# 1005088h/3d_object_detection

Hardware: AMD Instinct MI355X
Metric: point-cloud frames/sec end-to-end (voxelise→NMS), eight_20cm, 1x MI355X (higher is better)
Workload: dtype f32; 1 GPU; configs/eight_20cm.json, synthetic KITTI-shape 64-beam 20k-point clouds (mean 20000 points, one distinct cloud per frame of a step), independent frames (batch=1 semantics), random-init weights (InstanceNorm backbone), AABB NMS; `value`: clouds resident in HBM; frames_per_pass_per_gpu=32, engine_max_batch=32, parallelism=frame-sharded x1

## Files before the change

3d_object_detection_amd/_lib.py:

```python
import ctypes
import os

_HERE = os.path.dirname(os.path.abspath(__file__))
LIB_PATH = os.path.join(_HERE, "csrc", "libpp_hip.so")
PP_MAX_CLASSES = 12
PP_LOSS_TERMS = 21
PP_ASSIGN_MAX_GT = 4096
PP_AUG_MAX_BOXES = 256
PP_AUG_MAX_TRIES = 128
PP_AUG_PARAMS = 16

c_f = ctypes.c_float
c_i32 = ctypes.c_int32
c_i64 = ctypes.c_int64
c_p = ctypes.c_void_p


class PPConfig(ctypes.Structure):
    _fields_ = [
        ("voxel_size", c_f * 3),
        ("offset", c_f * 3),
        ("grid_size", c_i32 * 3),
        ("max_voxels", c_i32),
        ("max_num_points", c_i32),
# ... 23 lines not shown
    "pp_effective_precision": (ctypes.c_int, [c_p]),
    "pp_set_anchors": (ctypes.c_int, [c_p, c_p, c_p, c_i64]),
    "pp_voxelize": (ctypes.c_int, [c_p, c_p, ctypes.c_int, ctypes.c_int, c_p, c_p, c_p, c_p, c_p]),
    "pp_anchor_mask": (ctypes.c_int, [c_p, c_p, c_p, c_p, c_p]),
    "pp_pfn": (ctypes.c_int, [c_p, c_p, c_p, c_p, c_p, c_p, c_p]),
    "pp_scatter": (ctypes.c_int, [c_p, c_p, c_p, c_p, c_p, c_p]),
    "pp_backbone": (ctypes.c_int, [c_p, c_p, c_p, c_p]),
    "pp_head": (ctypes.c_int, [c_p, c_p, c_p, c_p, c_p, c_p]),
    "pp_postprocess": (ctypes.c_int, [c_p, c_p, c_p, c_p, c_p, c_p, c_p, ctypes.c_int, c_p]),
    "pp_select_candidates": (ctypes.c_int, [c_p, c_p, c_p, c_p, c_p, c_p, c_p, c_p, c_p]),
    "pp_infer_frame": (ctypes.c_int, [c_p, c_p, ctypes.c_int, c_p, c_p, ctypes.c_int, c_p]),
    "pp_infer_batch": (ctypes.c_int, [c_p, ctypes.POINTER(c_p), ctypes.POINTER(c_i32), ctypes.c_int, c_p, c_p, ctypes.c_int, c_p]),
    "pp_fetch_frame_tensor": (ctypes.c_int, [c_p, ctypes.c_int, ctypes.c_int, c_p, c_p]),
    "pp_set_head_defer": (ctypes.c_int, [c_p, ctypes.c_int]),
    "pp_head_defer_active": (ctypes.c_int, [c_p]),
    "pp_set_assign_thresholds": (ctypes.c_int, [c_p, c_p, c_p]),
    "pp_assign_targets": (ctypes.c_int, [c_p, c_p, c_p, c_p, ctypes.POINTER(c_i32), ctypes.c_int, c_p, c_p, c_p, c_p, c_p]),
    "pp_target_loss": (ctypes.c_int, [c_p, c_p, c_p, c_p, c_p, c_p, c_p, ctypes.c_int, c_p, c_p]),
    "pp_batch_loss": (ctypes.c_int, [c_p, c_p, c_p, ctypes.POINTER(c_i32), ctypes.c_int, c_p, c_p]),
    "pp_target_loss_grad": (ctypes.c_int, [c_p, c_p, c_p, c_p, c_p, c_p, c_p, ctypes.c_int, ctypes.c_int, c_f, c_p, c_p, c_p, c_p]),
    "pp_head_backward": (ctypes.c_int, [c_p, c_p, c_p, c_p, c_p, ctypes.c_int, c_p, c_p, c_p, c_p, c_p, c_p, c_p, c_p]),
    "pp_update_head_weights": (ctypes.c_int, [c_p, c_p, c_p, c_p, c_p, c_p, c_p, c_p]),
    "pp_augment_draw": (ctypes.c_int, [c_p, ctypes.c_uint64, ctypes.c_uint32, ctypes.POINTER(c_i64), ctypes.c_int, ctypes.c_int,
                                       ctypes.POINTER(c_i32), ctypes.c_int, c_p, c_p, c_p, c_p, c_p]),
    "pp_augment_noise": (ctypes.c_int, [c_p, c_p, c_p, c_p, c_p, c_p, ctypes.c_int, ctypes.POINTER(c_i32), ctypes.c_int, c_p, c_p, c_p, c_p]),
    "pp_augment_boxes": (ctypes.c_int, [c_p, c_p, c_p, c_p, c_p, c_p, c_p, c_p, ctypes.POINTER(c_i32), ctypes.c_int, c_p, c_p, c_p, c_p, c_p]),
    "pp_augment_points": (ctypes.c_int, [c_p, c_p, c_p, ctypes.POINTER(c_i32), c_p, c_p, c_p, c_p, c_p, ctypes.POINTER(c_i32), ctypes.c_int,
                                         c_p, c_p]),
    "pp_box_decode": (ctypes.c_int, [c_p, c_p, c_p, c_i64, c_p]),
    "pp_corners2d": (ctypes.c_int, [c_p, c_p, c_p, c_p, c_i64, c_p]),
# ... 48 lines not shown
```

3d_object_detection_amd/csrc/conv.hip:

```cpp
#include <algorithm>
#include <type_traits>
#include <cmath>
#include <cstdio>
#include <cstdlib>
#include <cstring>
#include <unistd.h>
#include "pp_common.h"
#include "conv_common.h"

namespace {

using namespace ppc;

template <int KS, int STRIDE, int TW, int WM, int WN, int MT, int NT, int BTX, int KC, int EPI>
struct ConvCfg {
    static constexpr int TH = 16 / TW;
    static constexpr int TILES = WN * NT;
    static constexpr int BTY = TILES / BTX;
    static constexpr int PW = BTX * TW, PH = BTY * TH;
    static constexpr int IW = (PW - 1) * STRIDE + KS, IH = (PH - 1) * STRIDE + KS;
    static constexpr int HALF = (IW + 1) / 2;
    static constexpr int iwp()
    {
        int v = IW;
// ... 2796 lines not shown
        for (Layer& L : net->layers) {
            int rc = 0;
            {
                const int h = H >> L.level, w = W >> L.level;
                const int hin = (L.kind == 0 && L.stride == 2) ? h * 2 : h, win = (L.kind == 0 && L.stride == 2) ? w * 2 : w;
                if (!can_tune && net->eff_prec == 0) L.var = pick_variant(L.kind, L.stride, L.up, (L.kind == 2) ? head_rows(ctx->cfg.num_anchor_per_loc) : (L.kind == 1 ? L.cout * L.up * L.up : L.cout), h, w, ctx->cfg.num_anchor_per_loc == 9);
                rc = autotune_layer(ctx, L, hin, win, h, w, tin, tout, verbose, can_tune);
                if (rc) { if (tin) { (void)hipFree(tin - W6_FRONT_PAD); (void)hipFree(tout); } return rc; }
            }
            PP_HIP(hipFuncSetAttribute((const void*)L.var.kern, hipFuncAttributeMaxDynamicSharedMemorySize,
                                       (int)layer_lds(L.var, L.cin)));
            if (L.var.kern2) PP_HIP(hipFuncSetAttribute((const void*)L.var.kern2, hipFuncAttributeMaxDynamicSharedMemorySize, (int)L.var.lds));
            rc = pack_layer(ctx, L);
            if (rc) { if (tin) { (void)hipFree(tin - W6_FRONT_PAD); (void)hipFree(tout); } return rc; }
        }
        {
            const Layer& head = net->layers.back();
            net->defer_ok = net->eff_prec == 0 && na == 9 && head.var.family == Family::Gemm1x1 && head.var.prec == 0 && head.var.io16 == 0;
            if (net->defer_ok) {
                const int rc = autotune_head_cls(ctx, tin, verbose, can_tune);
                if (rc) { if (tin) { (void)hipFree(tin - W6_FRONT_PAD); (void)hipFree(tout); } return rc; }
            }
        }
        if (tin) { PP_HIP(hipDeviceSynchronize()); (void)hipFree(tin - W6_FRONT_PAD); (void)hipFree(tout); tune_cache_save(); }
        if (net->up16)
            for (const Layer& L : net->layers)
                if ((L.kind == 1 && L.var.io16 != 3) || (L.kind == 2 && L.var.io16 != 1) ||
                    (L.kind == 0 && L.var.io16 != ((L.stride == 2 && L.level == 0) ? 2 : 3)))
                    return pp_fail(ctx, PP_E_STATE, "fp16s: a layer did not get a 16-bit-tensor tiling (PP_FORCE_VARIANT?)");
    }
// ... 73 lines not shown
    if (bx > 64) bx = 64;
    hipLaunchKernelGGL(norm_relu_stats, dim3(bx, C, B), dim3(256), 0, stream, x, y, C, HW, pre.mode, pre.acc, pre.scale,
                       pre.shift, pre.inv_n, 1e-3f, stat, (size_t)C * HW, STAT_FS, x16, y16);
    PP_HIP(hipGetLastError());
    return 0;
}

}

int pp_run_backbone(pp_ctx* ctx, const float* canvas, int nb, hipStream_t stream, const int32_t* pmap, const float* feat)
{
    pp_net* net = (pp_net*)ctx->net;
    const int H = ctx->H, W = ctx->W;
    if ((H % 4) || (W % 4)) return pp_fail(ctx, PP_E_ARG, "backbone: BEV grid must be a multiple of 8 in x and y");
    if (nb < 1 || nb > ctx->max_batch) return pp_fail(ctx, PP_E_ARG, "backbone: batch exceeds cfg.max_batch");
    if (ctx->cfg.norm_kind == 0) PP_HIP(hipMemsetAsync(net->stats, 0, STAT_FS * sizeof(double) * nb, stream));
    NormRef raw;
    const float* x = canvas;
    int Hin = ctx->gx, Win = ctx->gy;
    size_t li = 0;
    const int up_coff[3] = {0, 64, 192};
    const size_t up_fs = (size_t)320 * H * W;
    for (int b = 0; b < 3; ++b) {
        const int c = kC[b];
        const int h = H >> b, w = W >> b;
        const size_t cnt = (size_t)h * w;
        float** Bf = net->buf[b];
        int rc;
        if ((rc = launch_conv(ctx, net->layers[li++], x, Hin, Win, Bf[0], nullptr, raw, stat_slot(ctx, site_block(b, 0)), c, h, w, stream,
                              nullptr, nullptr, nb, 0, 0, b == 0 ? pmap : nullptr, b == 0 ? feat : nullptr))) return rc;
        if ((rc = pp_stage_mark(ctx, stream, PP_ST_NORM))) return rc;
        if ((rc = launch_norm_relu(ctx, Bf[0], Bf[1], c, (int)cnt, norm_ref(ctx, site_block(b, 0), c, 0, cnt),
                                   stat_slot(ctx, site_block(b, 1)), stream, nb, net->up16 ? 1 : 0, net->up16 ? 1 : 0))) return rc;
        if ((rc = pp_stage_mark(ctx, stream, PP_ST_CONV))) return rc;
        float* cur = Bf[1];
        float* spare[3] = {Bf[0], Bf[2], Bf[3]};
        const int nunits = (b == 0) ? 2 : 3;
        for (int u = 0; u < nunits; ++u) {
            const int nl = (u == nunits - 1) ? 0 : 1;
            const bool last = (u == nunits - 1);
            float* t1 = spare[0];
            float* t2 = spare[1];
            double* out_stat = last ? nullptr : stat_slot(ctx, site_block(b, 1 + 2 * (u + 1)));
            if (nl == 1) {
// ... 180 lines not shown
    switch (kind) {
    case 0: src = ctx->f_cls + frame * A; bytes = A * 4; break;
    case 1: src = ctx->f_box + frame * A * 7; bytes = A * 28; break;
    case 2: src = ctx->f_dir + frame * A * 2; bytes = A * 8; break;
    case 3: src = ctx->f_mask + frame * A; bytes = A; break;
    case 4: {
        NormRef pre = norm_ref(ctx, 7, 320, 0, HW);
        if (pre.mode == PRE_STATS) pre.acc += (size_t)frame * STAT_FS;
        const float* src_ = net->up16 ? reinterpret_cast<const float*>(reinterpret_cast<const _Float16*>(net->up) + (size_t)frame * 320 * HW)
                                      : net->up + (size_t)frame * 320 * HW;
        return launch_norm_relu(ctx, src_, (float*)dst, 320, (int)HW, pre, nullptr, stream, 1, net->up16 ? 1 : 0);
    }
    case 5: src = ctx->f_feat + frame * mv * 64; bytes = mv * 64 * 4; break;
    case 6: src = ctx->f_coors + frame * mv * 3; bytes = mv * 12; break;
    case 7: src = ctx->f_num + frame * 4; bytes = 4; break;
    default: return pp_fail(ctx, PP_E_ARG, "pp_fetch_frame_tensor: unknown kind");
    }
    PP_HIP(hipMemcpyAsync(dst, src, bytes, hipMemcpyDeviceToDevice, stream));
    return 0;
}

extern "C" int pp_profile_begin(pp_ctx* ctx)
{
    if (!ctx) return PP_E_ARG;
    ctx->prof_on = true;
    ctx->prof_used = 0;
    return 0;
}

extern "C" int pp_profile_end(pp_ctx* ctx, double* avg_ms, int32_t* launches, double* flops)
// ... 92 lines not shown
```

3d_object_detection_amd/csrc/pp_api.hip:

```cpp
#include <cmath>
#include <cstdio>
#include <cstdlib>
#include <cstring>
#include "pp_common.h"

static std::string g_create_err;

int pp_fail_hip(pp_ctx* ctx, hipError_t e, const char* what, const char* file, int line)
{
    char buf[512];
    snprintf(buf, sizeof(buf), "%s failed: %s (%s:%d)", what, hipGetErrorString(e), file, line);
    if (ctx) ctx->err = buf; else g_create_err = buf;
    (void)hipGetLastError();
    return -(int)e;
}

int pp_fail(pp_ctx* ctx, int code, const char* msg)
{
    if (ctx) ctx->err = msg; else g_create_err = msg;
    return code;
}

extern "C" const char* pp_last_error(pp_ctx* ctx) { return ctx ? ctx->err.c_str() : g_create_err.c_str(); }
extern "C" int pp_version(void) { return 4; }
// ... 77 lines not shown
    PP_HIP(dalloc(&ctx->f_voxels, mv * c.max_num_points * c.num_point_features));
    PP_HIP(dalloc(&ctx->f_coors, mv * 3));
    PP_HIP(dalloc(&ctx->f_npts, mv));
    PP_HIP(dalloc(&ctx->f_num, 4 * (size_t)ctx->max_batch));
    PP_HIP(dalloc(&ctx->f_feat, mv * 64));
    PP_HIP(dalloc(&ctx->f_canvas, (size_t)64 * ctx->gx * ctx->gy));
    PP_HIP(dalloc(&ctx->f_pmap, (size_t)ctx->max_batch * ctx->gx * ctx->gy));
    size_t HW = (size_t)ctx->H * ctx->W;
    size_t Amax = HW * c.num_anchor_per_loc * ctx->max_batch;
    PP_HIP(dalloc(&ctx->f_mask, Amax));
    PP_HIP(dalloc(&ctx->f_cls, Amax));
    PP_HIP(dalloc(&ctx->f_box, Amax * 7));
    PP_HIP(dalloc(&ctx->f_dir, Amax * 2));
    int rc = pp_net_create(ctx);
    if (rc) return rc;
    rc = pp_post_create(ctx);
    return rc;
}

extern "C" pp_ctx* pp_create(int device, const pp_config* cfg)
{
    if (!cfg) { pp_fail(nullptr, PP_E_ARG, "pp_create: null config"); return nullptr; }
    if (cfg->grid_size[2] != 1 || cfg->grid_size[0] < 2 || cfg->grid_size[1] < 2 || (cfg->grid_size[0] & 1) ||
        (cfg->grid_size[1] & 1)) {
        pp_fail(nullptr, PP_E_ARG, "pp_create: grid must be [gx,gy,1] with even gx,gy (multiples of 8 for the backbone)");
        return nullptr;
    }
    if (cfg->max_voxels <= 0 || cfg->max_num_points <= 0 || cfg->max_points <= 0 || cfg->num_classes <= 0 ||
        cfg->num_classes > PP_MAX_CLASSES || cfg->nms_pre_max <= 0 || cfg->nms_pre_max > 4096 ||
        cfg->nms_post_max <= 0 || cfg->nms_post_max > cfg->nms_pre_max || cfg->nms_post_max > 1024 || cfg->max_batch < 0 ||
        cfg->max_batch > 64) {
        pp_fail(nullptr, PP_E_ARG, "pp_create: size out of range");
        return nullptr;
    }
    pp_ctx* ctx = new pp_ctx();
    ctx->cfg = *cfg;
    ctx->max_batch = cfg->max_batch > 0 ? cfg->max_batch : 1;
    ctx->cfg.max_batch = ctx->max_batch;
    ctx->device = device;
    ctx->gx = cfg->grid_size[0];
    ctx->gy = cfg->grid_size[1];
    ctx->H = ctx->gx / 2;
    ctx->W = ctx->gy / 2;
    if (const char* e = getenv("PP_HEAD_DEFER")) ctx->head_defer_env_off = e[0] == '0';
    ctx->head_defer = !ctx->head_defer_env_off;
    int rc = create_impl(ctx);
    if (rc) {
        g_create_err = ctx->err;
        pp_destroy(ctx);
        return nullptr;
    }
    return ctx;
}

int pp_build_tables(pp_ctx* ctx)
{
    if (ctx->tab_A == ctx->A) return 0;
    const pp_config& c = ctx->cfg;
    const size_t mv = (size_t)c.max_voxels;
    const size_t vs = mv * c.max_num_points * c.num_point_features;
// ... 16 lines not shown
        pp_post_frame& q = post[b];
        PP_SET(q.cls, ctx->f_cls + b * A); PP_SET(q.box, ctx->f_box + b * A * 7); PP_SET(q.dir, ctx->f_dir + b * A * 2); PP_SET(q.mask, ctx->f_mask + b * A);
        pp_post_fill_table(ctx, b, &q);
    }
    PP_HIP(hipMemcpy(ctx->d_pre, pre.data(), sizeof(pp_pre_frame) * pre.size(), hipMemcpyHostToDevice));
    PP_HIP(hipMemcpy(ctx->d_post, post.data(), sizeof(pp_post_frame) * post.size(), hipMemcpyHostToDevice));
    ctx->tab_A = ctx->A;
    return 0;
}

extern "C" void pp_destroy(pp_ctx* ctx)
{
    if (!ctx) return;
    (void)hipSetDevice(ctx->device);
    pp_net_destroy(ctx);
    pp_post_destroy(ctx);
    pp_assign_destroy(ctx);
    pp_train_destroy(ctx);
    for (pp_slot& S : ctx->slot) {
        void* sp[] = {S.cell_first, S.pt_cell, S.pt_rank, S.wave_cnt, S.occ};
        for (void* q : sp)
            if (q) (void)hipFree(q);
    }
    if (ctx->d_pre) (void)hipFree(ctx->d_pre);
    if (ctx->d_post) (void)hipFree(ctx->d_post);
    void* ptrs[] = {ctx->anchors, ctx->rect_x, ctx->rect_y, ctx->rects, ctx->pfn_w, ctx->pfn_scale, ctx->pfn_shift,
                    ctx->f_voxels, ctx->f_coors, ctx->f_npts, ctx->f_num, ctx->f_feat, ctx->f_canvas, ctx->f_mask, ctx->f_pmap,
                    ctx->f_cls, ctx->f_box, ctx->f_dir};
    for (void* p : ptrs)
        if (p) (void)hipFree(p);
// ... 43 lines not shown
                      *b = find_w(ctx, p + "1.bias", 64), *rm = find_w(ctx, p + "1.running_mean", 64),
                      *rv = find_w(ctx, p + "1.running_var", 64);
    if (!w || !g || !b || !rm || !rv) return pp_fail(ctx, PP_E_NAME, "pp_commit_weights: PFN tensors missing or mis-shaped");
    float wT[9 * 64], sc[64], sh[64];
    for (int c = 0; c < 64; ++c) {
        for (int k = 0; k < 9; ++k) wT[k * 64 + c] = w->data[c * 9 + k];
        double s = (double)g->data[c] / std::sqrt((double)rv->data[c] + 1e-5);
        sc[c] = (float)s;
        sh[c] = (float)((double)b->data[c] - (double)rm->data[c] * s);
    }
    PP_HIP(hipMemcpy(ctx->pfn_w, wT, sizeof(wT), hipMemcpyHostToDevice));
    PP_HIP(hipMemcpy(ctx->pfn_scale, sc, sizeof(sc), hipMemcpyHostToDevice));
    PP_HIP(hipMemcpy(ctx->pfn_shift, sh, sizeof(sh), hipMemcpyHostToDevice));
    int rc = pp_net_commit(ctx);
    if (rc) return rc;
    ctx->weights_ready = true;
    ++ctx->commit_gen;
    return 0;
}

extern "C" int pp_set_anchors(pp_ctx* ctx, const float* anchors_h, const int32_t* rects_h, int64_t A)
{
    if (!ctx || !anchors_h || !rects_h || A <= 0) return pp_fail(ctx, PP_E_ARG, "pp_set_anchors: bad argument");
    PP_HIP(hipSetDevice(ctx->device));
    const int H = ctx->H, W = ctx->W;
    const int64_t HW = (int64_t)H * W;
    if (A % HW != 0 || A / HW != ctx->cfg.num_anchor_per_loc)
        return pp_fail(ctx, PP_E_ARG, "pp_set_anchors: A must be num_anchor_per_loc * (gx/2) * (gy/2)");
    for (int i = 0; i < 4 * A; ++i) {
        int lim = (i & 1) ? ctx->gy : ctx->gx;
// ... 31 lines not shown
```

3d_object_detection_amd/csrc/pp_common.h:

```cpp
#pragma once
#include <hip/hip_runtime.h>
#include <stdint.h>
#include <map>
#include <string>
#include <vector>
#include "../../include/pp_hip.h"

#define PP_EMPTY 0x7F7F7F7F

#define PP_HIP(call)                                                         \
    do {                                                                     \
        hipError_t e_ = (call);                                              \
        if (e_ != hipSuccess) return pp_fail_hip(ctx, e_, #call, __FILE__, __LINE__); \
    } while (0)

#if defined(__HIP_DEVICE_COMPILE__)
#define PP_GP __attribute__((address_space(1)))
#else
#define PP_GP
#endif
#define PP_SET(dst, src) dst = (decltype(dst))(src)
struct pp_pre_frame {
    int32_t PP_GP *pt_cell, *cell_first, *wave_cnt, *pt_rank, *slots, *scalars, *occ;
    float PP_GP* voxels;
// ... 74 lines not shown
    std::vector<hipEvent_t> stage_ev;
    std::vector<int> stage_id;
    std::vector<hipStream_t> stage_stream;
    size_t stage_used = 0;
    int last_nb = 0;
    bool asg_thr_set = false;
    float asg_thr_m[PP_MAX_CLASSES] = {}, asg_thr_u[PP_MAX_CLASSES] = {};
    void* asg = nullptr;
    uint64_t commit_gen = 0;
    void* trn = nullptr;
    bool head_defer = true;
    bool head_defer_env_off = false;
    bool head_stale = false;
    int stale_nb = 0;
    hipStream_t stale_stream = nullptr;
};
enum { PP_ST_VOXELIZE = 0, PP_ST_MASK = 1, PP_ST_PFN = 2, PP_ST_CONV = 3, PP_ST_NORM = 4, PP_ST_HEAD = 5, PP_ST_POST = 6 ,
       PP_ST_POST_TOPK = 7 , PP_ST_POST_NMS = 8 , PP_ST_COUNT = 12 };
int pp_stage_mark(pp_ctx* ctx, hipStream_t stream, int id);

int pp_fail_hip(pp_ctx* ctx, hipError_t e, const char* what, const char* file, int line);
int pp_fail(pp_ctx* ctx, int code, const char* msg);

int pp_net_create(pp_ctx* ctx);
void pp_net_destroy(pp_ctx* ctx);
int pp_net_commit(pp_ctx* ctx);
int pp_post_create(pp_ctx* ctx);
int pp_voxelize_slot(pp_ctx* ctx, int s, const float* pts, int n, int nfeat, float* voxels, int32_t* coors, int32_t* npts,
                     int32_t* num_pillars, hipStream_t stream);
int pp_anchor_mask_slot(pp_ctx* ctx, int s, const int32_t* coors, const int32_t* num_pillars, uint8_t* mask, hipStream_t stream);
// ... 7 lines not shown
int pp_anchor_mask_group(pp_ctx* ctx, int b0, int g, hipStream_t stream);
int pp_pfn_pmap_group(pp_ctx* ctx, int b0, int g, hipStream_t stream);
int pp_postprocess_group(pp_ctx* ctx, int b0, int g, float* det, int32_t* det_count, int nms_mode, hipStream_t stream,
                         int defer_nb = 0);
int pp_run_head_fused(pp_ctx* ctx, float* cls, float* box, float* dir, int nb, hipStream_t stream);
bool pp_head_defer_on(pp_ctx* ctx);
int pp_run_head_cls(pp_ctx* ctx, float* cls, int nb, hipStream_t stream);
int pp_head_materialise(pp_ctx* ctx, hipStream_t stream);
struct pp_head_gather {
    const float* w; int bm, bmp, K;
    const float* bias_perm;
    const float* in; size_t in_fs; int HW;
    int pre; const double* pre_acc; size_t pre_fs; double pre_inv_n; const float *pre_scale, *pre_shift; size_t aff_fs; float eps;
};
int pp_net_head_gather(pp_ctx* ctx, int nb, pp_head_gather* g);
void pp_post_destroy(pp_ctx* ctx);
void pp_assign_destroy(pp_ctx* ctx);
void pp_train_destroy(pp_ctx* ctx);
struct pp_head_image {
    float *w = nullptr, *bias = nullptr, *bias_perm = nullptr;
    std::vector<int32_t> wmap, bmap, bpmap;
};
int pp_net_head_image(pp_ctx* ctx, pp_head_image* img);

static inline int pp_div_up(int64_t a, int64_t b) { return (int)((a + b - 1) / b); }
```

3d_object_detection_amd/engine.py:

```python
import ctypes
import os
import weakref

import numpy as np
import torch

from . import _lib

F32 = np.float32

DETECT_CLASSES = ["vehicle", "pedestrian", "cyclist"]
CLASS_TABLE = {
    "vehicle": dict(sizes=[[4.6, 2.10, 1.8], [7.5, 2.6, 2.9], [12.6, 2.9, 3.8]], rotations=[0, 1.5707963267948966],
                    matched_threshold=0.6, unmatched_threshold=0.45),
    "pedestrian": dict(sizes=[[0.96874749, 0.9645992, 1.81212425]], rotations=[0],
                       matched_threshold=0.45, unmatched_threshold=0.25),
    "cyclist": dict(sizes=[[2.02032733, 0.98075615, 1.72027404]], rotations=[0, 1.5707963267948966],
                    matched_threshold=0.5, unmatched_threshold=0.25),
}
NUM_ANCHOR_PER_LOC = 9


def class_table_of(config):
    tab = config.get("class_table")
# ... 178 lines not shown
        if changed and self.weights_loaded:
            with torch.cuda.device(self.device):
                _lib.check(self.lib.pp_commit_weights(self.ctx), self.ctx, "pp_commit_weights")

    def effective_precision(self):
        v = self.lib.pp_effective_precision(self.ctx)
        return None if v < 0 else {n: k for k, n in self.PRECISIONS.items()}[v]

    def set_head_defer(self, on):
        _lib.check(self.lib.pp_set_head_defer(self.ctx, 1 if on else 0), self.ctx, "pp_set_head_defer")
        self.head_defer = bool(on) and not self._defer_env_off

    def head_defer_active(self):
        return bool(self.lib.pp_head_defer_active(self.ctx))

    def load_state_dict(self, sd):
        for k, v in sd.items():
            if k.endswith("num_batches_tracked"):
                continue
            a = v.detach().cpu().numpy() if isinstance(v, torch.Tensor) else np.asarray(v)
            a = np.ascontiguousarray(a, dtype=F32)
            shape = (ctypes.c_int64 * max(a.ndim, 1))(*a.shape)
            _lib.check(self.lib.pp_load_weights(self.ctx, k.encode(), a.ctypes.data_as(ctypes.c_void_p), shape, a.ndim),
                       self.ctx, "pp_load_weights(" + k + ")")
        with torch.cuda.device(self.device):
            _lib.check(self.lib.pp_commit_weights(self.ctx), self.ctx, "pp_commit_weights")
        self.weights_loaded = True

    def _t(self, shape, dtype):
        return torch.empty(shape, dtype=dtype, device=self.device)
# ... 157 lines not shown
        rows = self.cfg.num_classes * self.cfg.nms_post_max
        if det is None:
            det = torch.zeros((nb, rows, 9), dtype=torch.float32, device=self.device)
            cnt = torch.zeros((nb, 1 + _lib.PP_MAX_CLASSES), dtype=torch.int32, device=self.device)
        ptrs = (ctypes.c_void_p * nb)(*[p.data_ptr() if p.numel() else _ptr(p).value for p in points_list])
        ns = (ctypes.c_int32 * nb)(*[int(p.shape[0]) for p in points_list])
        with torch.cuda.device(self.device):
            _lib.check(self.lib.pp_infer_batch(self.ctx, ptrs, ns, nb, _ptr(det), _ptr(cnt), int(nms_mode), _stream()),
                       self.ctx, "pp_infer_batch")
        return det, cnt

    def fetch(self, frame, what):
        kinds = {"cls": (0, (self.A,), torch.float32), "box": (1, (self.A, 7), torch.float32), "dir": (2, (self.A, 2), torch.float32),
                 "mask": (3, (self.A,), torch.uint8), "rpn": (4, (320, self.H, self.W), torch.float32),
                 "feat": (5, (self.max_voxels, 64), torch.float32), "coors": (6, (self.max_voxels, 3), torch.int32),
                 "num": (7, (1,), torch.int32)}
        kind, shape, dtype = kinds[what]
        out = torch.empty(shape, dtype=dtype, device=self.device)
        with torch.cuda.device(self.device):
            _lib.check(self.lib.pp_fetch_frame_tensor(self.ctx, int(frame), kind, _ptr(out), _stream()), self.ctx, "pp_fetch_frame_tensor")
        return out

    def _gt_args(self, gt_boxes, gt_classes, gt_offsets, nb, what):
        G = int(gt_boxes.shape[0]) if gt_boxes.dim() == 2 else -1
        gt_boxes = _chk(gt_boxes, torch.float32, (G, 7), what + ": gt_boxes")
        gt_classes = _chk(gt_classes, torch.int32, (G,), what + ": gt_classes")
        off = [int(v) for v in gt_offsets]
        if not 1 <= nb <= self.max_batch:
            raise ValueError(f"{what}: {nb} frames, max_batch is {self.max_batch}")
        if len(off) != nb + 1 or off[0] != 0 or off[-1] != G or any(b < a for a, b in zip(off, off[1:])):
            raise ValueError(f"{what}: gt offsets must be {nb + 1} non-decreasing values from 0 to {G}")
# ... 248 lines not shown
```

include/pp_hip.h:

```cpp
#ifndef PP_HIP_H
#define PP_HIP_H
#include <stdint.h>

#ifdef __cplusplus
extern "C" {
#endif

#define PP_MAX_CLASSES 12
#define PP_E_ARG 1
#define PP_E_STATE 2
#define PP_E_NAME 3

typedef struct pp_ctx pp_ctx;

typedef struct pp_config {
    float voxel_size[3];
    float offset[3];
    int32_t grid_size[3];
    int32_t max_voxels;
    int32_t max_num_points;
    int32_t num_point_features;
    int32_t max_points;
    int32_t num_anchor_per_loc;
    int32_t num_classes;
// ... 40 lines not shown

int pp_select_candidates(pp_ctx* ctx, const float* cls, const float* box, const float* dir, const uint8_t* mask,
                         int32_t* idx, float* score, int32_t* count, void* stream);

int pp_infer_frame(pp_ctx* ctx, const float* pts, int n, float* det, int32_t* det_count, int nms_mode, void* stream);

#define PP_DET_COUNT_STRIDE (1 + PP_MAX_CLASSES)
int pp_infer_batch(pp_ctx* ctx, const float* const* pts_h, const int32_t* n_h, int nb, float* det, int32_t* det_count,
                   int nms_mode, void* stream);

int pp_fetch_frame_tensor(pp_ctx* ctx, int frame, int kind, void* dst, void* stream);

int pp_set_head_defer(pp_ctx* ctx, int on);
int pp_head_defer_active(pp_ctx* ctx);

#define PP_ASSIGN_MAX_GT 4096
#define PP_LOSS_TERMS 21
int pp_set_assign_thresholds(pp_ctx* ctx, const float* matched_h, const float* unmatched_h);
int pp_assign_targets(pp_ctx* ctx, const uint8_t* mask, const float* gt, const int32_t* gt_cls, const int32_t* gt_off_h, int nb,
                      int32_t* labels, float* bbox_targets, float* outside_w, int32_t* dir_targets, void* stream);
int pp_target_loss(pp_ctx* ctx, const float* cls, const float* box, const float* dir, const int32_t* labels,
                   const float* bbox_targets, const int32_t* dir_targets, int nb, double* terms, void* stream);
int pp_batch_loss(pp_ctx* ctx, const float* gt, const int32_t* gt_cls, const int32_t* gt_off_h, int nb, double* terms, void* stream);

int pp_target_loss_grad(pp_ctx* ctx, const float* cls, const float* box, const float* dir, const int32_t* labels,
                        const float* bbox_targets, const int32_t* dir_targets, int nb, int batch_div, float grad_scale, float* dcls,
                        float* dbox, float* ddir, void* stream);
int pp_head_backward(pp_ctx* ctx, const float* rpn_out, const float* dcls, const float* dbox, const float* ddir, int nb, float* dw_cls,
                     float* dw_box, float* dw_dir, float* db_cls, float* db_box, float* db_dir, float* dx, void* stream);
int pp_update_head_weights(pp_ctx* ctx, const float* w_cls, const float* b_cls, const float* w_box, const float* b_box, const float* w_dir,
// ... 58 lines not shown
```

Measured before the change: 1012 frames/s.

## Add sparse gather-based first backbone conv over active output pixels

Replaces the dense stride-2 3x3 first backbone convolution with a sparse path. It ballots the output pixels whose receptive field contains an occupied pillar, compacts them into a per-frame list with gather tables, and runs an MFMA kernel that reads pillar features straight from the voxel feature buffer. It writes only the active outputs after zeroing the output plane, and accumulates the norm statistics inside the same kernel. The path is on by default for fp32 and adds three launches plus a memset, with results capped at a fixed active-pixel capacity.

```diff
diff --git a/3d_object_detection_amd/_lib.py b/3d_object_detection_amd/_lib.py
--- a/3d_object_detection_amd/_lib.py
+++ b/3d_object_detection_amd/_lib.py
@@ -61,6 +61,7 @@
     "pp_fetch_frame_tensor": (ctypes.c_int, [c_p, ctypes.c_int, ctypes.c_int, c_p, c_p]),
     "pp_set_head_defer": (ctypes.c_int, [c_p, ctypes.c_int]),
     "pp_head_defer_active": (ctypes.c_int, [c_p]),
+    "pp_set_sparse_conv1": (ctypes.c_int, [c_p, ctypes.c_int]),
     "pp_set_assign_thresholds": (ctypes.c_int, [c_p, c_p, c_p]),
     "pp_assign_targets": (ctypes.c_int, [c_p, c_p, c_p, c_p, ctypes.POINTER(c_i32), ctypes.c_int, c_p, c_p, c_p, c_p, c_p]),
     "pp_target_loss": (ctypes.c_int, [c_p, c_p, c_p, c_p, c_p, c_p, c_p, ctypes.c_int, c_p, c_p]),
diff --git a/3d_object_detection_amd/csrc/conv.hip b/3d_object_detection_amd/csrc/conv.hip
--- a/3d_object_detection_amd/csrc/conv.hip
+++ b/3d_object_detection_amd/csrc/conv.hip
@@ -2834,6 +2834,7 @@
             rc = pack_layer(ctx, L);
             if (rc) { if (tin) { (void)hipFree(tin - W6_FRONT_PAD); (void)hipFree(tout); } return rc; }
         }
+        ctx->sc1_kc = (net->layers[0].var.family == Family::Direct && net->layers[0].var.kc == 8) ? 8 : 4;
         {
             const Layer& head = net->layers.back();
             net->defer_ok = net->eff_prec == 0 && na == 9 && head.var.family == Family::Gemm1x1 && head.var.prec == 0 && head.var.io16 == 0;
@@ -2937,6 +2938,7 @@
     const int H = ctx->H, W = ctx->W;
     if ((H % 4) || (W % 4)) return pp_fail(ctx, PP_E_ARG, "backbone: BEV grid must be a multiple of 8 in x and y");
     if (nb < 1 || nb > ctx->max_batch) return pp_fail(ctx, PP_E_ARG, "backbone: batch exceeds cfg.max_batch");
+    ctx->sc1_last_nb = 0;
     if (ctx->cfg.norm_kind == 0) PP_HIP(hipMemsetAsync(net->stats, 0, STAT_FS * sizeof(double) * nb, stream));
     NormRef raw;
     const float* x = canvas;
@@ -2950,7 +2952,10 @@
         const size_t cnt = (size_t)h * w;
         float** Bf = net->buf[b];
         int rc;
-        if ((rc = launch_conv(ctx, net->layers[li++], x, Hin, Win, Bf[0], nullptr, raw, stat_slot(ctx, site_block(b, 0)), c, h, w, stream,
+        if (b == 0 && pmap && net->eff_prec == 0 && pp_sc1_usable(ctx)) {
+            ++li;
+            if ((rc = pp_sc1_run(ctx, pmap, feat, Bf[0], stat_slot(ctx, site_block(0, 0)), STAT_FS, nb, stream))) return rc;
+        } else if ((rc = launch_conv(ctx, net->layers[li++], x, Hin, Win, Bf[0], nullptr, raw, stat_slot(ctx, site_block(b, 0)), c, h, w, stream,
                               nullptr, nullptr, nb, 0, 0, b == 0 ? pmap : nullptr, b == 0 ? feat : nullptr))) return rc;
         if ((rc = pp_stage_mark(ctx, stream, PP_ST_NORM))) return rc;
         if ((rc = launch_norm_relu(ctx, Bf[0], Bf[1], c, (int)cnt, norm_ref(ctx, site_block(b, 0), c, 0, cnt),
@@ -3161,6 +3166,7 @@
     case 5: src = ctx->f_feat + frame * mv * 64; bytes = mv * 64 * 4; break;
     case 6: src = ctx->f_coors + frame * mv * 3; bytes = mv * 12; break;
     case 7: src = ctx->f_num + frame * 4; bytes = 4; break;
+    case 8: return pp_sc1_fetch_list(ctx, frame, dst, stream);
     default: return pp_fail(ctx, PP_E_ARG, "pp_fetch_frame_tensor: unknown kind");
     }
     PP_HIP(hipMemcpyAsync(dst, src, bytes, hipMemcpyDeviceToDevice, stream));
diff --git a/3d_object_detection_amd/csrc/pp_api.hip b/3d_object_detection_amd/csrc/pp_api.hip
--- a/3d_object_detection_amd/csrc/pp_api.hip
+++ b/3d_object_detection_amd/csrc/pp_api.hip
@@ -115,6 +115,8 @@
     PP_HIP(dalloc(&ctx->f_dir, Amax * 2));
     int rc = pp_net_create(ctx);
     if (rc) return rc;
+    rc = pp_sc1_create(ctx);
+    if (rc) return rc;
     rc = pp_post_create(ctx);
     return rc;
 }
@@ -145,6 +147,8 @@
     ctx->W = ctx->gy / 2;
     if (const char* e = getenv("PP_HEAD_DEFER")) ctx->head_defer_env_off = e[0] == '0';
     ctx->head_defer = !ctx->head_defer_env_off;
+    if (const char* e = getenv("PP_SPARSE_CONV1")) ctx->sparse_conv1_env_off = e[0] == '0';
+    ctx->sparse_conv1 = !ctx->sparse_conv1_env_off;
     int rc = create_impl(ctx);
     if (rc) {
         g_create_err = ctx->err;
@@ -191,6 +195,7 @@
     if (!ctx) return;
     (void)hipSetDevice(ctx->device);
     pp_net_destroy(ctx);
+    pp_sc1_destroy(ctx);
     pp_post_destroy(ctx);
     pp_assign_destroy(ctx);
     pp_train_destroy(ctx);
@@ -264,6 +269,7 @@
     PP_HIP(hipMemcpy(ctx->pfn_shift, sh, sizeof(sh), hipMemcpyHostToDevice));
     int rc = pp_net_commit(ctx);
     if (rc) return rc;
+    if ((rc = pp_sc1_commit(ctx))) return rc;
     ctx->weights_ready = true;
     ++ctx->commit_gen;
     return 0;
diff --git a/3d_object_detection_amd/csrc/pp_common.h b/3d_object_detection_amd/csrc/pp_common.h
--- a/3d_object_detection_amd/csrc/pp_common.h
+++ b/3d_object_detection_amd/csrc/pp_common.h
@@ -112,6 +112,11 @@
     bool head_stale = false;
     int stale_nb = 0;
     hipStream_t stale_stream = nullptr;
+    bool sparse_conv1 = true;
+    bool sparse_conv1_env_off = false;
+    void* sc1 = nullptr;
+    int sc1_kc = 4;
+    int sc1_last_nb = 0;
 };
 enum { PP_ST_VOXELIZE = 0, PP_ST_MASK = 1, PP_ST_PFN = 2, PP_ST_CONV = 3, PP_ST_NORM = 4, PP_ST_HEAD = 5, PP_ST_POST = 6 ,
        PP_ST_POST_TOPK = 7 , PP_ST_POST_NMS = 8 , PP_ST_COUNT = 12 };
@@ -149,6 +154,12 @@
     int pre; const double* pre_acc; size_t pre_fs; double pre_inv_n; const float *pre_scale, *pre_shift; size_t aff_fs; float eps;
 };
 int pp_net_head_gather(pp_ctx* ctx, int nb, pp_head_gather* g);
+int pp_sc1_create(pp_ctx* ctx);
+void pp_sc1_destroy(pp_ctx* ctx);
+int pp_sc1_commit(pp_ctx* ctx);
+bool pp_sc1_usable(pp_ctx* ctx);
+int pp_sc1_run(pp_ctx* ctx, const int32_t* pmap, const float* feat, float* out, double* stat, size_t stat_fs, int nb, hipStream_t stream);
+int pp_sc1_fetch_list(pp_ctx* ctx, int frame, void* dst, hipStream_t stream);
 void pp_post_destroy(pp_ctx* ctx);
 void pp_assign_destroy(pp_ctx* ctx);
 void pp_train_destroy(pp_ctx* ctx);
diff --git a/3d_object_detection_amd/csrc/sparse_conv1.hip b/3d_object_detection_amd/csrc/sparse_conv1.hip
--- /dev/null
+++ b/3d_object_detection_amd/csrc/sparse_conv1.hip
@@ -0,0 +1,317 @@
+#include <algorithm>
+#include <cstring>
+#include "pp_common.h"
+#include "conv_common.h"
+
+namespace {
+
+using namespace ppc;
+
+constexpr unsigned SC1_PARK = 0x80000000u;
+constexpr int SC1_NT = 4;
+constexpr int SC1_WAVE_PX = 16 * SC1_NT;
+constexpr int SC1_W_FLOATS = 9 * 64 * 64;
+
+struct Sc1 {
+    float* w = nullptr;
+    int kc = 4;
+    uint64_t* words = nullptr;
+    int32_t* bcnt = nullptr;
+    int32_t* list = nullptr;
+    uint32_t* tab = nullptr;
+    int32_t* count = nullptr;
+    int cap = 0, cap_pad = 0, nblk = 0;
+    bool weights = false;
+};
+
+struct Sc1P {
+    const int32_t* pmap; size_t pmap_fs;
+    const float* feat; size_t feat_fs; unsigned feat_bytes;
+    const float* w;
+    float* out; size_t out_fs;
+    double* stat; size_t stat_fs;
+    uint64_t* words; int32_t* bcnt; int32_t* list; uint32_t* tab; int32_t* count;
+    int Hin, Win, Hout, Wout, cap, cap_pad, nblk, max_voxels;
+};
+
+__global__ void __launch_bounds__(256) sc1_ballot_b(const Sc1P p)
+{
+    __shared__ int wc[4];
+    const int f = blockIdx.z;
+    const int32_t* __restrict__ gmap = p.pmap + (size_t)f * p.pmap_fs;
+    const int pix = blockIdx.x * 256 + threadIdx.x;
+    bool act = false;
+    if (pix < p.Hout * p.Wout) {
+        const int oy = pix / p.Wout, ox = pix - oy * p.Wout;
+#pragma unroll
+        for (int ky = 0; ky < 3; ++ky) {
+            const int iy = 2 * oy - 1 + ky;
+#pragma unroll
+            for (int kx = 0; kx < 3; ++kx) {
+                const int ix = 2 * ox - 1 + kx;
+                if (iy >= 0 && iy < p.Hin && ix >= 0 && ix < p.Win) act |= gmap[(size_t)iy * p.Win + ix] >= 0;
+            }
+        }
+    }
+    const uint64_t b = __ballot(act);
+    const int wave = threadIdx.x >> 6;
+    if ((threadIdx.x & 63) == 0) {
+        p.words[((size_t)f * p.nblk + blockIdx.x) * 4 + wave] = b;
+        wc[wave] = __popcll(b);
+    }
+    __syncthreads();
+    if (threadIdx.x == 0) p.bcnt[(size_t)f * p.nblk + blockIdx.x] = wc[0] + wc[1] + wc[2] + wc[3];
+}
+
+__global__ void __launch_bounds__(256) sc1_write_b(const Sc1P p)
+{
+    __shared__ int red[4];
+    const int f = blockIdx.z, blk = blockIdx.x, tid = threadIdx.x, lane = tid & 63, wave = tid >> 6;
+    const uint64_t* __restrict__ wd = p.words + ((size_t)f * p.nblk + blk) * 4;
+    const int32_t* __restrict__ bc = p.bcnt + (size_t)f * p.nblk;
+    const uint64_t w0 = wd[0], w1 = wd[1], w2 = wd[2], w3 = wd[3];
+    const int c0 = __popcll(w0), c1 = __popcll(w1), c2 = __popcll(w2), c3 = __popcll(w3);
+    const int own = c0 + c1 + c2 + c3;
+    const bool last = blk == p.nblk - 1;
+    if (own == 0 && !last) return;
+    int s = 0;
+    for (int i = tid; i < blk; i += 256) s += bc[i];
+#pragma unroll
+    for (int d = 1; d < 64; d <<= 1) s += __shfl_xor(s, d);
+    if (lane == 0) red[wave] = s;
+    __syncthreads();
+    const int prefix = red[0] + red[1] + red[2] + red[3];
+    if (last && tid == 0) {
+        const int total = prefix + own;
+        p.count[f] = total < p.cap ? total : p.cap;
+    }
+    const uint64_t mw = wave == 0 ? w0 : wave == 1 ? w1 : wave == 2 ? w2 : w3;
+    const int before = prefix + (wave > 0 ? c0 : 0) + (wave > 1 ? c1 : 0) + (wave > 2 ? c2 : 0);
+    const int rank = before + __popcll(mw & ((1ull << lane) - 1ull));
+    if (!((mw >> lane) & 1ull) || rank >= p.cap) return;
+    const int pix = blk * 256 + tid;
+    const int oy = pix / p.Wout, ox = pix - oy * p.Wout;
+    const int32_t* __restrict__ gmap = p.pmap + (size_t)f * p.pmap_fs;
+    p.list[(size_t)f * p.cap_pad + rank] = pix;
+    uint32_t* __restrict__ tb = p.tab + (size_t)f * 9 * p.cap_pad + rank;
+#pragma unroll
+    for (int ky = 0; ky < 3; ++ky) {
+        const int iy = 2 * oy - 1 + ky;
+#pragma unroll
+        for (int kx = 0; kx < 3; ++kx) {
+            const int ix = 2 * ox - 1 + kx;
+            int id = -1;
+            if (iy >= 0 && iy < p.Hin && ix >= 0 && ix < p.Win) id = gmap[(size_t)iy * p.Win + ix];
+            tb[(size_t)(ky * 3 + kx) * p.cap_pad] = (id >= 0 && id < p.max_voxels) ? ((unsigned)id * 256u) ^ SC1_PARK : 0u;
+        }
+    }
+}
+
+template <int KC> constexpr int sc1_c4(int q) { return KC == 8 ? (q / 18) * 2 + (q % 18) % 2 : q / 9; }
+template <int KC> constexpr int sc1_tap(int q) { return KC == 8 ? (q % 18) / 2 : q % 9; }
+
+template <int KC>
+__global__ void __launch_bounds__(256) sc1_gather(const Sc1P p)
+{
+    constexpr int NT = SC1_NT;
+    const int f = blockIdx.z;
+    const int lane = threadIdx.x & 63, n = lane & 15, kq = lane >> 4;
+    const int wv = blockIdx.x * 4 + (threadIdx.x >> 6);
+    const int cnt = p.count[f];
+    const int e0 = wv * SC1_WAVE_PX;
+    if (e0 >= cnt) return;
+    const __amdgpu_buffer_rsrc_t rf = __builtin_amdgcn_make_buffer_rsrc(const_cast<float*>(p.feat + (size_t)f * p.feat_fs), 0, p.feat_bytes, 0x00020000);
+    const __amdgpu_buffer_rsrc_t rw = __builtin_amdgcn_make_buffer_rsrc(const_cast<float*>(p.w), 0, SC1_W_FLOATS * 4, 0x00020000);
+    const __amdgpu_buffer_rsrc_t rt = __builtin_amdgcn_make_buffer_rsrc(p.tab + (size_t)f * 9 * p.cap_pad, 0, (unsigned)p.cap_pad * 36u, 0x00020000);
+    const __amdgpu_buffer_rsrc_t rl = __builtin_amdgcn_make_buffer_rsrc(p.list + (size_t)f * p.cap_pad, 0, (unsigned)p.cap_pad * 4u, 0x00020000);
+    bool valid[NT];
+    unsigned eo[NT];
+#pragma unroll
+    for (int t = 0; t < NT; ++t) {
+        valid[t] = e0 + t * 16 + n < cnt;
+        eo[t] = valid[t] ? (unsigned)(e0 + t * 16 + n) * 4u : SC1_PARK;
+    }
+    const unsigned tap_b = (unsigned)p.cap_pad * 4u;
+    unsigned vo[NT][9];
+#pragma unroll
+    for (int tap = 0; tap < 9; ++tap)
+#pragma unroll
+        for (int t = 0; t < NT; ++t) vo[t][tap] = (__builtin_amdgcn_raw_buffer_load_b32(rt, eo[t], (unsigned)tap * tap_b, 0) ^ SC1_PARK) + (unsigned)kq * 4u;
+
+    f32x4 a[2][4];
+    float b[2][4][NT];
+    f32x4 acc[4][NT];
+#pragma unroll
+    for (int i = 0; i < 4; ++i)
+#pragma unroll
+        for (int t = 0; t < NT; ++t) acc[i][t] = (f32x4){0.f, 0.f, 0.f, 0.f};
+
+#define SC1_LOAD_OPS(G, SET)                                                                                   \
+    pp_steps<0, 4>([&](auto S_) {                                                                              \
+        constexpr int q_ = (G) * 4 + decltype(S_)::value, sl_ = decltype(S_)::value;                           \
+        _Pragma("unroll") for (int t = 0; t < NT; ++t)                                                         \
+            b[SET][sl_][t] = __builtin_bit_cast(float, __builtin_amdgcn_raw_buffer_load_b32(rf, vo[t][sc1_tap<KC>(q_)] + sc1_c4<KC>(q_) * 16, 0, 0)); \
+        a[SET][sl_] = __builtin_bit_cast(f32x4, __builtin_amdgcn_raw_buffer_load_b128(rw, (unsigned)lane * 16u, q_ * 1024, 0)); \
+    });
+    SC1_LOAD_OPS(0, 0)
+    pp_steps<0, 36>([&](auto G) {
+        constexpr int g_ = decltype(G)::value;
+        constexpr int cur = g_ & 1;
+        if constexpr (g_ + 1 < 36) SC1_LOAD_OPS(g_ + 1, cur ^ 1)
+        __builtin_amdgcn_sched_barrier(0);
+#pragma unroll
+        for (int s = 0; s < 4; ++s)
+#pragma unroll
+            for (int i = 0; i < 4; ++i)
+#pragma unroll
+                for (int t = 0; t < NT; ++t)
+                    acc[i][t] = __builtin_amdgcn_mfma_f32_16x16x4f32(a[cur][s][i], b[cur][s][t], acc[i][t], 0, 0, 0);
+        __builtin_amdgcn_sched_barrier(0);
+    });
+#undef SC1_LOAD_OPS
+
+    const unsigned plane_b = (unsigned)(p.Hout * p.Wout) * 4u;
+    const __amdgpu_buffer_rsrc_t ro = __builtin_amdgcn_make_buffer_rsrc(p.out + (size_t)f * p.out_fs, 0, plane_b * 64u, 0x00020000);
+#pragma unroll
+    for (int t = 0; t < NT; ++t) {
+        const unsigned pix = __builtin_amdgcn_raw_buffer_load_b32(rl, eo[t], 0, 0);
+        const unsigned oo = valid[t] ? pix * 4u + (unsigned)kq * 4u * plane_b : SC1_PARK;
+#pragma unroll
+        for (int i = 0; i < 4; ++i)
+#pragma unroll
+            for (int r = 0; r < 4; ++r) {
+                const float x = acc[i][t][r];
+                __builtin_amdgcn_raw_buffer_store_b32(__builtin_bit_cast(unsigned, x), ro, oo, (unsigned)(i * 16 + r) * plane_b, 0);
+            }
+    }
+    if (p.stat) {
+        double* __restrict__ gs = p.stat + (size_t)f * p.stat_fs + (size_t)(wv % NREP) * 64 * 2;
+#pragma unroll
+        for (int i = 0; i < 4; ++i)
+#pragma unroll
+            for (int r = 0; r < 4; ++r) {
+                double s = 0.0, q = 0.0;
+#pragma unroll
+                for (int t = 0; t < NT; ++t) { const float x = acc[i][t][r]; const float xx = x * x; s += (double)x; q += (double)xx; }
+#pragma unroll
+                for (int d = 1; d < 16; d <<= 1) { s += __shfl_xor(s, d); q += __shfl_xor(q, d); }
+                if (n == 0) {
+                    double* dst = gs + (size_t)(i * 16 + kq * 4 + r) * 2;
+                    atomicAdd(dst, s);
+                    atomicAdd(dst + 1, q);
+                }
+            }
+    }
+}
+
+template <typename T>
+hipError_t sc1_alloc(T** q, size_t count) { return hipMalloc((void**)q, count * sizeof(T) + 256); }
+
+}
+
+int pp_sc1_create(pp_ctx* ctx)
+{
+    Sc1* S = new Sc1();
+    ctx->sc1 = S;
+    const size_t HW = (size_t)ctx->H * ctx->W, mb = (size_t)ctx->max_batch;
+    const size_t cap = std::min((size_t)4 * ctx->cfg.max_voxels, HW);
+    S->cap = (int)cap;
+    S->cap_pad = (int)((cap + SC1_WAVE_PX - 1) / SC1_WAVE_PX) * SC1_WAVE_PX;
+    S->nblk = pp_div_up((int64_t)HW, 256);
+    PP_HIP(sc1_alloc(&S->w, (size_t)SC1_W_FLOATS));
+    PP_HIP(sc1_alloc(&S->words, mb * S->nblk * 4));
+    PP_HIP(sc1_alloc(&S->bcnt, mb * S->nblk));
+    PP_HIP(sc1_alloc(&S->list, mb * S->cap_pad));
+    PP_HIP(sc1_alloc(&S->tab, mb * 9 * S->cap_pad));
+    PP_HIP(sc1_alloc(&S->count, mb));
+    PP_HIP(hipMemset(S->list, 0, mb * S->cap_pad * sizeof(int32_t)));
+    PP_HIP(hipMemset(S->tab, 0, mb * 9 * S->cap_pad * sizeof(uint32_t)));
+    PP_HIP(hipMemset(S->count, 0, mb * sizeof(int32_t)));
+    return 0;
+}
+
+void pp_sc1_destroy(pp_ctx* ctx)
+{
+    Sc1* S = (Sc1*)ctx->sc1;
+    if (!S) return;
+    void* ptrs[] = {S->w, S->words, S->bcnt, S->list, S->tab, S->count};
+    for (void* q : ptrs)
+        if (q) (void)hipFree(q);
+    delete S;
+    ctx->sc1 = nullptr;
+}
+
+int pp_sc1_commit(pp_ctx* ctx)
+{
+    Sc1* S = (Sc1*)ctx->sc1;
+    S->weights = false;
+    auto it = ctx->host_w.find("rpn.block1.0.weight");
+    if (it == ctx->host_w.end() || it->second.data.size() != (size_t)SC1_W_FLOATS)
+        return pp_fail(ctx, PP_E_NAME, "missing/mis-shaped weight rpn.block1.0.weight");
+    const std::vector<float>& w = it->second.data;
+    std::vector<float> img((size_t)SC1_W_FLOATS);
+    S->kc = ctx->sc1_kc == 8 ? 8 : 4;
+    for (int q = 0; q < 144; ++q) {
+        const int c4 = S->kc == 8 ? sc1_c4<8>(q) : sc1_c4<4>(q), tap = S->kc == 8 ? sc1_tap<8>(q) : sc1_tap<4>(q);
+        for (int lane = 0; lane < 64; ++lane)
+            for (int i = 0; i < 4; ++i) {
+                const int co = 16 * i + (lane & 15), ci = 4 * c4 + (lane >> 4);
+                img[((size_t)q * 64 + lane) * 4 + i] = w[((size_t)co * 64 + ci) * 9 + tap];
+            }
+    }
+    PP_HIP(hipMemcpy(S->w, img.data(), img.size() * sizeof(float), hipMemcpyHostToDevice));
+    S->weights = true;
+    return 0;
+}
+
+bool pp_sc1_usable(pp_ctx* ctx)
+{
+    const Sc1* S = (const Sc1*)ctx->sc1;
+    return ctx->sparse_conv1 && S && S->weights && (size_t)64 * ctx->H * ctx->W * 4 < 0x7F000000ull &&
+           (size_t)ctx->cfg.max_voxels * 256 < 0x7F000000ull;
+}
+
+int pp_sc1_run(pp_ctx* ctx, const int32_t* pmap, const float* feat, float* out, double* stat, size_t stat_fs, int nb, hipStream_t stream)
+{
+    Sc1* S = (Sc1*)ctx->sc1;
+    const size_t HW = (size_t)ctx->H * ctx->W;
+    ctx->sc1_last_nb = 0;
+    PP_HIP(hipMemsetAsync(out, 0, (size_t)nb * 64 * HW * sizeof(float), stream));
+    for (int b0 = 0; b0 < nb; b0 += PP_GROUP) {
+        const int g = nb - b0 < PP_GROUP ? nb - b0 : PP_GROUP;
+        Sc1P p;
+        memset(&p, 0, sizeof(p));
+        p.pmap_fs = (size_t)ctx->gx * ctx->gy; p.pmap = pmap + b0 * p.pmap_fs;
+        p.feat_fs = (size_t)ctx->cfg.max_voxels * 64; p.feat = feat + b0 * p.feat_fs;
+        p.feat_bytes = (unsigned)(p.feat_fs * 4);
+        p.w = S->w;
+        p.out_fs = 64 * HW; p.out = out + b0 * p.out_fs;
+        p.stat_fs = stat_fs; p.stat = stat ? stat + b0 * stat_fs : nullptr;
+        p.words = S->words + (size_t)b0 * S->nblk * 4; p.bcnt = S->bcnt + (size_t)b0 * S->nblk;
+        p.list = S->list + (size_t)b0 * S->cap_pad; p.tab = S->tab + (size_t)b0 * 9 * S->cap_pad; p.count = S->count + b0;
+        p.Hin = ctx->gx; p.Win = ctx->gy; p.Hout = ctx->H; p.Wout = ctx->W;
+        p.cap = S->cap; p.cap_pad = S->cap_pad; p.nblk = S->nblk; p.max_voxels = ctx->cfg.max_voxels;
+        hipLaunchKernelGGL(sc1_ballot_b, dim3(S->nblk, 1, g), dim3(256), 0, stream, p);
+        hipLaunchKernelGGL(sc1_write_b, dim3(S->nblk, 1, g), dim3(256), 0, stream, p);
+        hipLaunchKernelGGL(S->kc == 8 ? sc1_gather<8> : sc1_gather<4>, dim3(pp_div_up(S->cap_pad, 4 * SC1_WAVE_PX), 1, g), dim3(256), 0, stream, p);
+    }
+    PP_HIP(hipGetLastError());
+    ctx->sc1_last_nb = nb;
+    return 0;
+}
+
+int pp_sc1_fetch_list(pp_ctx* ctx, int frame, void* dst, hipStream_t stream)
+{
+    const Sc1* S = (const Sc1*)ctx->sc1;
+    if (!S || frame >= ctx->sc1_last_nb) return pp_fail(ctx, PP_E_STATE, "pp_fetch_frame_tensor: the last pass did not build an active list for this frame");
+    PP_HIP(hipMemcpyAsync(dst, S->count + frame, sizeof(int32_t), hipMemcpyDeviceToDevice, stream));
+    PP_HIP(hipMemcpyAsync((int32_t*)dst + 1, S->list + (size_t)frame * S->cap_pad, (size_t)S->cap * sizeof(int32_t), hipMemcpyDeviceToDevice, stream));
+    return 0;
+}
+
+extern "C" int pp_set_sparse_conv1(pp_ctx* ctx, int on)
+{
+    if (!ctx) return PP_E_ARG;
+    ctx->sparse_conv1 = on && !ctx->sparse_conv1_env_off;
+    return 0;
+}
diff --git a/3d_object_detection_amd/engine.py b/3d_object_detection_amd/engine.py
--- a/3d_object_detection_amd/engine.py
+++ b/3d_object_detection_amd/engine.py
@@ -216,6 +216,9 @@
     def head_defer_active(self):
         return bool(self.lib.pp_head_defer_active(self.ctx))
 
+    def set_sparse_conv1(self, on):
+        _lib.check(self.lib.pp_set_sparse_conv1(self.ctx, 1 if on else 0), self.ctx, "pp_set_sparse_conv1")
+
     def load_state_dict(self, sd):
         for k, v in sd.items():
             if k.endswith("num_batches_tracked"):
@@ -403,7 +406,7 @@
         kinds = {"cls": (0, (self.A,), torch.float32), "box": (1, (self.A, 7), torch.float32), "dir": (2, (self.A, 2), torch.float32),
                  "mask": (3, (self.A,), torch.uint8), "rpn": (4, (320, self.H, self.W), torch.float32),
                  "feat": (5, (self.max_voxels, 64), torch.float32), "coors": (6, (self.max_voxels, 3), torch.int32),
-                 "num": (7, (1,), torch.int32)}
+                 "num": (7, (1,), torch.int32), "active": (8, (1 + min(4 * self.max_voxels, self.H * self.W),), torch.int32)}
         kind, shape, dtype = kinds[what]
         out = torch.empty(shape, dtype=dtype, device=self.device)
         with torch.cuda.device(self.device):
diff --git a/include/pp_hip.h b/include/pp_hip.h
--- a/include/pp_hip.h
+++ b/include/pp_hip.h
@@ -78,6 +78,8 @@
 int pp_set_head_defer(pp_ctx* ctx, int on);
 int pp_head_defer_active(pp_ctx* ctx);
 
+int pp_set_sparse_conv1(pp_ctx* ctx, int on);
+
 #define PP_ASSIGN_MAX_GT 4096
 #define PP_LOSS_TERMS 21
 int pp_set_assign_thresholds(pp_ctx* ctx, const float* matched_h, const float* unmatched_h);
```

Result: faster. 1045 frames/s, median of 6 (+3.2%).
